# YoungSeng/QPGesture

Hardware: AMD Instinct MI355X
Metric: matched gesture frames/sec (GestureKNN) (higher is better)
Workload: dtype split-f16 products / f64 block sums + f64 re-evaluation; 1 GPU; 1 x 24 s clip (M=6 windows, Q=48 steps, 1440 frames each) per job vs speaker-10-class DB N_db=2048 windows (53248 candidates), shipped mode wavlm_feat(f32-bounded/f64-exact)+text(f32)+phase; n_db=2048, windows_per_clip=6, clips=1, clips_per_gpu=1, feature_dtype=f32, audio_precision=mixed, encode_batch=0, clips_in_flight=1, parallelism=single GPU, unsharded DB

## Files before the change

### include/qpg.h

```cpp
#ifndef QPG_H
#define QPG_H

#include <stddef.h>
#include <stdint.h>

#ifdef __cplusplus
extern "C" {
#endif

#define QPG_OK 0
#define QPG_EINVAL (-1)
#define QPG_EHIP (-2)
#define QPG_EUNSUP (-3)

typedef struct qpg_ctx qpg_ctx;

int qpg_version(void);
const char* qpg_build_id(void);
int qpg_ctx_create(int device, qpg_ctx** out);
int qpg_dev_kernarg(void);
int qpg_ctx_destroy(qpg_ctx* ctx);
#define QPG_OPT_GATE_DEDUP_FROM_CHAINS 0
#define QPG_OPT_TAKES_STAGES 1
#define QPG_OPT_NOPHASE_STAGES 2
// ... 8 lines not shown
int qpg_wavlm_resample_f32(qpg_ctx*, void* stream, const float* x, int64_t N, int Tin, int F, int Tout, float* out);

int qpg_frame_norm2_f64(qpg_ctx*, void* stream, const float* x, int64_t rows, int F, double* out);

int qpg_audio_cand_norm2(qpg_ctx*, void* stream, const double* fn2, int N, int T, const int32_t* cand_t,
                         int G, int n_taps, int tap_stride, double* cn2);

int qpg_l2_normalize_rows_f32(qpg_ctx*, void* stream, const float* x, int64_t rows, int D, float* out);
int qpg_text_pack_queries_f32(qpg_ctx*, void* stream, const float* x, int M, int R, int D, const int32_t* q_win,
                              const int32_t* q_row, int Q, float* out);


int qpg_audio_pack_queries(qpg_ctx*, void* stream, const float* qbase, int M, int T, int F,
                           const int32_t* q_win, const int32_t* q_t, int Q, int n_taps, int tap_stride,
                           float* q32, double* qn2);

int qpg_audio_cosine_f64(qpg_ctx*, void* stream, const float* base, int N, int T, int F,
                         const int32_t* cand_t, int G, int n_taps, int tap_stride, const double* cn2,
                         const float* q32, const double* qn2, int Q, double* D, int64_t ldD);
int qpg_audio_cosine_f64_h(qpg_ctx*, void* stream, const void* base_f16, int N, int T, int F,
                           const int32_t* cand_t, int G, int n_taps, int tap_stride, const double* cn2,
                           const float* q32, const double* qn2, int Q, double* D, int64_t ldD);

#define QPG_AUDIO_MX_ERR 2.05e-6
int qpg_audio_cosine_mx(qpg_ctx*, void* stream, const float* base, int N, int T, int F, const int32_t* cand_t, int G,
                        int n_taps, int tap_stride, const double* cn2, const float* q32, const double* qn2, int Q,
                        void* D, int d_is_f32, int64_t ldD, int32_t* stats);

int qpg_audio_cosine_mx_h(qpg_ctx*, void* stream, const void* base_f16, int N, int T, int F, const int32_t* cand_t, int G,
                          int n_taps, int tap_stride, const double* cn2, const float* q32, const double* qn2, int Q,
                          void* D, int d_is_f32, int64_t ldD, int32_t* stats);

#define QPG_AUDIO_HL_ERR 1.3e-6
int qpg_audio_hl_supported(int T, int F, int G, int n_taps, int tap_stride, int cand_step);
int qpg_audio_pack_queries_hl(qpg_ctx*, void* stream, const float* qbase, int M, int T, int F, const int32_t* q_win,
                              const int32_t* q_t, int Q, int n_taps, int tap_stride, float* q32, double* qn2, void* image,
                              int64_t image_bytes);
int64_t qpg_audio_hl_db_bytes(int N, int F);
int64_t qpg_audio_hl_query_bytes(int Q, int F);
int qpg_audio_hl_pack_db(qpg_ctx*, void* stream, const float* base, int N, int T, int F, int G, int n_taps, int tap_stride,
                         int cand_step, void* image, int64_t image_bytes);
int qpg_audio_hl_pack_queries(qpg_ctx*, void* stream, const float* q32, int Q, int F, void* image, int64_t image_bytes);
int qpg_clip_pack_hl(qpg_ctx*, void* stream, const float* qbase, int M, int T, int F, const int32_t* q_win,
                     const int32_t* q_t, int Q, int n_taps, int tap_stride, float* q32, double* qn2, void* image,
                     int64_t image_bytes, const float* text_ctx, int Mt, int R, int Dt, const int32_t* tq_win,
                     const int32_t* tq_row, int Qt, float* qn_out, void* cols_image, int64_t cols_bytes);
int qpg_audio_cosine_hl(qpg_ctx*, void* stream, const void* db_image, int N, int F, int G, const double* cn2,
                        const void* q_image, const double* qn2, int Q, void* D, int d_is_f32, int64_t ldD, int32_t* stats);
int qpg_audio_hl1_supported(int T, int F, int G, int n_taps, int tap_stride, int cand_step);
int64_t qpg_audio_hl1_db_bytes(int N, int F);
int qpg_audio_hl1_pack_db(qpg_ctx*, void* stream, const void* base_f16, int N, int T, int F, int G, int n_taps,
                          int tap_stride, int cand_step, void* image, int64_t image_bytes);
int qpg_audio_cosine_hl1(qpg_ctx*, void* stream, const void* db_image, int N, int F, int G, const double* cn2,
                         const void* q_image, const double* qn2, int Q, void* D, int d_is_f32, int64_t ldD, int32_t* stats);
int qpg_probe_mfma_f16_tile(qpg_ctx*, void* stream, const void* a, const void* b, const float* c, int tiles, float* out);

int qpg_text_pack_candidates_f32(qpg_ctx*, void* stream, const float* x, int N, int R, int Dm,
                                 const int32_t* cand_r, int G, float* xt);

int qpg_text_cosine_f32(qpg_ctx*, void* stream, const float* xt, int64_t C, int Dm, const float* qn, int Q,
                        float* D, int64_t ldD);

int64_t qpg_text_percode_ws_bytes(int64_t C, int Q, int K, int tiles_per_chunk);
int qpg_text_percode_f32(qpg_ctx*, void* stream, const float* xt, int64_t C, int Dm, const int16_t* cand_code, int K,
                         const float* qn, int Q, int tiles_per_chunk, int32_t idx_base, float absent, void* ws,
                         int64_t ws_bytes, float* out_dist, int32_t* out_idx, int16_t* out_rank, int32_t* out_nn);
int qpg_text_pack_candidates_f16(qpg_ctx*, void* stream, const float* x, int N, int R, int Dm, const int32_t* cand_r,
                                 int G, void* xh, float* nrm);
int qpg_text_percode_f16(qpg_ctx*, void* stream, const void* xh, const float* nrm, int64_t C, int Dm,
                         const int16_t* cand_code, int K, const float* qn, int Q, int32_t idx_base, float absent,
                         void* ws, int64_t ws_bytes, float* out_dist, int32_t* out_idx, int16_t* out_rank,
                         int32_t* out_nn);

int64_t qpg_hl_rows_bytes(int64_t R, int D);
int64_t qpg_hl_cols_bytes(int Q, int D);
int qpg_hl_pack_rows(qpg_ctx*, void* stream, const float* xs, int64_t R, int D, void* image, int64_t image_bytes);
int qpg_hl_pack_cols(qpg_ctx*, void* stream, const float* qn, int Q, int D, void* image, int64_t image_bytes);
int qpg_hl_prepare_queries(qpg_ctx*, void* stream, const float* q, int Q, int D, float* qn_out, void* cols_image,
                           int64_t image_bytes, float* qperm_out);
int qpg_hl_gemm_distance(qpg_ctx*, void* stream, const void* rows_image, int64_t R, int D, const void* cols_image, int Q,
                         float* Dm, int64_t ldD, float* tile_min, int64_t ldT);
int qpg_hl_gemm_tilemin(qpg_ctx*, void* stream, const void* rows_image, int64_t R, int D, const void* cols_image, int Q,
                        float band, float* tile_min, uint16_t* tile_mask, int64_t ldT);
int qpg_hl_gemm_tilemin_h(qpg_ctx*, void* stream, const void* rows_image, int64_t R, int D, const void* cols_image, int Q,
                          float band, float* tile_min_t, uint16_t* tile_mask_t, int64_t ldQ);
int qpg_perm32_rows_f32(qpg_ctx*, void* stream, const float* x, int64_t R, int D, float* y);
int qpg_percode_select_bycode_f32(qpg_ctx*, void* stream, const float* tile_min_t, const uint16_t* tile_mask_t, int64_t ldQ,
                                  int Q, int64_t R, const int16_t* row_code, const int32_t* row_index,
                                  const int32_t* zero_row, const int32_t* code_tile, int K, float band,
                                  const float* qn_perm, const float* xs_perm, int D, float absent, float* out_dist,
                                  int32_t* out_idx, int16_t* out_rank, int32_t* out_nn, int32_t* stats, int32_t idx_base);
int qpg_percode_select_sorted_f32(qpg_ctx*, void* stream, const float* Dm, int64_t ldD, const float* tile_min,
                                  const uint16_t* tile_mask , int64_t ldT,
                                  int Q, int64_t R, const int16_t* row_code, const int32_t* row_index,
                                  const int32_t* zero_row, const int32_t* code_tile, int K, float band, const float* qn,
                                  const float* xs, int D, float absent, float* out_dist, int32_t* out_idx,
                                  int16_t* out_rank, int32_t* out_nn, int32_t* stats, int32_t idx_base, int q_block,
                                  int64_t block_stride);

int qpg_wavvq_lev_f32(qpg_ctx*, void* stream, const int32_t* sym_db, int N, int T, const int32_t* cand_t, int G,
                      const int32_t* tap_off, int n_taps, const int32_t* sym_q, int Mq, int Tq,
                      const int32_t* q_win, const int32_t* q_t, int Q, float* D, int64_t ldD);

int qpg_percode_select_f64(qpg_ctx*, void* stream, const double* D, int64_t ldD, int Q, const int16_t* cand_code,
                           int64_t C, int K, double absent, int32_t idx_base, double* out_dist, int32_t* out_idx,
                           int16_t* out_rank, int q_block, int64_t block_stride);
int qpg_percode_select_f32(qpg_ctx*, void* stream, const float* D, int64_t ldD, int Q, const int16_t* cand_code,
                           int64_t C, int K, float absent, int32_t idx_base, float* out_dist, int32_t* out_idx,
                           int16_t* out_rank, int q_block, int64_t block_stride);

int qpg_percode_select_guarded_f64(qpg_ctx*, void* stream, const double* D, int64_t ldD, int Q, const int16_t* cand_code,
                                   int64_t C, int K, double absent, int32_t idx_base, double* out_dist, int32_t* out_idx,
                                   int16_t* out_rank, int q_block, int64_t block_stride, const float* base, int T, int F,
                                   const int32_t* cand_t, int G, int n_taps, int tap_stride, const float* q32, double eps,
                                   int32_t* stats, int base_is_f16);

int64_t qpg_percode_select_exact_ws_bytes(int Q, int64_t C, int K);
int qpg_percode_select_exact_f64(qpg_ctx*, void* stream, const double* D, int64_t ldD, int Q, const int16_t* cand_code,
                                 int64_t C, int K, double absent, int32_t idx_base, double* out_dist, int32_t* out_idx,
                                 int16_t* out_rank, int q_block, int64_t block_stride, const float* base, int T, int F,
                                 const int32_t* cand_t, int G, int n_taps, int tap_stride, const float* q32, double eps,
                                 int32_t* stats, int base_is_f16, void* ws, int64_t ws_bytes);

int qpg_percode_select_mixed_f64(qpg_ctx*, void* stream, const void* D, int d_is_f32, int64_t ldD, int Q, const int16_t* cand_code,
                                 int64_t C, int K, double absent, int32_t idx_base, double* out_dist, int32_t* out_idx,
                                 int16_t* out_rank, int q_block, int64_t block_stride, const float* base, int T, int F,
                                 const int32_t* cand_t, int G, int n_taps, int tap_stride, const float* q32,
                                 const double* qn2, const double* cn2, double eps1, double eps2, int32_t* stats,
                                 void* ws, int64_t ws_bytes, int base_is_f16);
int64_t qpg_percode_select_mixed_ws_bytes(int Q, int K);
int64_t qpg_percode_select_mixed_ws_stride(int K);
int qpg_percode_select_mixed_f64_cut(qpg_ctx*, void* stream, const void* D, int d_is_f32, int64_t ldD, int Q,
                                     const int16_t* cand_code, int64_t C, int K, double absent, int32_t idx_base,
                                     double* out_dist, int32_t* out_idx, int16_t* out_rank, int q_block, int64_t block_stride,
                                     const float* base, int T, int F, const int32_t* cand_t, int G, int n_taps,
                                     int tap_stride, const float* q32, const double* qn2, const double* cn2, double eps1,
                                     double eps2, int32_t* stats, void* ws, int64_t ws_bytes, int base_is_f16,
                                     const int16_t* pos_rank_t, const int16_t* freq_rank, int top_n, int probe);

int64_t qpg_merge_mixed_ws_bytes(int Q, int K, int fl_cap);
int qpg_merge_mixed_phase1_f64(qpg_ctx*, void* stream, const void* recv, int W, int64_t src_stride, int64_t dist_off,
                               int64_t idx_off, int Q, int K, double absent, double eps1, int R, void* req,
                               int64_t req_stride, void* ws, int64_t ws_bytes, int32_t* stats, int fl_cap,
                               int64_t flag_off);
int qpg_shard_refine_f64(qpg_ctx*, void* stream, const void* req_recv, int W, int64_t req_stride, int R, int q_stride,
                         int64_t cand_base, const float* base, int base_is_f16, int T, int F, const int32_t* cand_t, int G,
                         int n_taps, int tap_stride, const float* q32, const double* qn2, const double* cn2, void* resp,
                         int64_t resp_stride, int reference_arithmetic, int32_t* stats, int Rq);
int qpg_flags_stamp(qpg_ctx*, void* stream, void* buf, int nblk, int64_t stride, int64_t off, const int32_t* stats);
int qpg_flags_gather(qpg_ctx*, void* stream, const void* buf, int nblk, int64_t stride, int64_t off, int32_t* stats);
int qpg_merge_mixed_phase2_f64(qpg_ctx*, void* stream, const void* recv, int W, int64_t src_stride, int64_t idx_off, int Q,
                               int K, double absent, const void* ws, int64_t ws_bytes, const void* resp_recv,
                               int64_t resp_stride, double* out_dist, int32_t* out_idx, int16_t* out_rank, int32_t* stats,
                               int fl_cap, double eps2);

int qpg_merge_select_f64(qpg_ctx*, void* stream, const void* recv, int W, int64_t src_stride, int64_t dist_off,
                         int64_t idx_off, int Q, int K, double absent, double* out_dist, int32_t* out_idx,
                         int16_t* out_rank, double eps2, int32_t* stats);
int qpg_merge_select_f32(qpg_ctx*, void* stream, const void* recv, int W, int64_t src_stride, int64_t dist_off,
                         int64_t idx_off, int Q, int K, float absent, float* out_dist, int32_t* out_idx,
                         int16_t* out_rank);

int qpg_rank_rows_f64(qpg_ctx*, void* stream, const double* d, int Q, int K, int16_t* out);
int qpg_rank_rows_f32(qpg_ctx*, void* stream, const float* d, int Q, int K, int16_t* out);


// ... 365 lines not shown
```

### qpgesture_amd/csrc/qpg_audio_hl.hip

```cpp
#include "qpg_common.h"
#include <stdlib.h>

typedef _Float16 h8 __attribute__((ext_vector_type(8)));
typedef _Float16 h4 __attribute__((ext_vector_type(4)));

#define HL_ROWS 27
#define HL_SUB 3
#define HL_QC 48
#define HL_CT 6
#define HL_GQC (16 * HL_CT)
#define HL_KS 2
#define HL_PIECE 1024

template <int PJ>
__device__ __forceinline__ float xor_lanes_f(float v) {
  return __int_as_float(lane_xor<PJ>(__float_as_int(v)));
}
__device__ __forceinline__ f32x4 mfma_h(h8 a, h8 b, f32x4 c) {
  return __builtin_amdgcn_mfma_f32_16x16x32_f16(a, b, c, 0, 0, 0);
}

__device__ __forceinline__ void split_hl(float x, _Float16& h, _Float16& l) {
  h = (_Float16)x;
  const float r = x - (float)h;
// ... 220 lines not shown

__global__ __launch_bounds__(768) void hl_pack_queries_fused_kernel(const float* __restrict__ qbase, int M, int T, int F,
                                                                    const int32_t* __restrict__ q_win,
                                                                    const int32_t* __restrict__ q_t, int Q, int tap_stride,
                                                                    float* __restrict__ q32, double* __restrict__ qn2,
                                                                    _Float16* __restrict__ image,
                                                                    int32_t* __restrict__ qexp) {
  hl_pack_query_block(blockIdx.x, threadIdx.x, qbase, M, T, F, q_win, q_t, Q, tap_stride, q32, qn2, image, qexp);
}

struct ClipPackText {
  const float* ctx;
  const int32_t* q_win;
  const int32_t* q_row;
  int R, Dt, Qt;
  float* qn;
  _Float16* image;
  int32_t* qexp;
};

__global__ __launch_bounds__(768) void hl_pack_clip_kernel(const float* __restrict__ qbase, int M, int T, int F,
                                                           const int32_t* __restrict__ q_win,
                                                           const int32_t* __restrict__ q_t, int Q, int tap_stride,
                                                           float* __restrict__ q32, double* __restrict__ qn2,
                                                           _Float16* __restrict__ image, int32_t* __restrict__ qexp,
                                                           int n_aud, ClipPackText tx) {
  const int tid = threadIdx.x;
  if ((int)blockIdx.x < n_aud) {
    hl_pack_query_block(blockIdx.x, tid, qbase, M, T, F, q_win, q_t, Q, tap_stride, q32, qn2, image, qexp);
    return;
  }
  const int qi = (int)blockIdx.x - n_aud;
  const int D = tx.Dt;
  extern __shared__ __attribute__((aligned(16))) float rowbuf[];
  __shared__ float n_s;
  const bool live = qi < tx.Qt;
  const float* p = live ? tx.ctx + ((int64_t)tx.q_win[qi] * tx.R + tx.q_row[qi]) * D : tx.ctx;
  if (tid < 4) {
    const float n = einsum_norm_f32(p, D, tid);
    if (tid == 0) n_s = n;
  }
  __syncthreads();
  const float n = n_s;
  float m = 0.f;
  for (int e = tid; e < D; e += 768) {
    const float v = live ? f_div(p[e], n) : 0.f;
    rowbuf[e] = v;
    if (live) tx.qn[(int64_t)qi * D + e] = v;
    m = fmaxf(m, fabsf(v));
  }
  const int e_q = hl_block_exponent<12>(m);
  if (live && tid == 0) tx.qexp[qi] = e_q;
  const float sc = ldexpf(1.0f, e_q);
  const int KB = D / 32, K8 = D / 8;
  for (int k8 = tid; k8 < K8; k8 += 768) {
    const int k = k8 * 8;
    h8 hh, ll;
    hl_split8<false>(rowbuf + k, sc, hh, ll);
    hl_store_col_piece(tx.image, qi, HL_GQC, KB, k, 0, hh, ll);
  }
}

struct HlArgs {
  const _Float16* db;
  const _Float16* qi;
  const int32_t* meta;
  const int32_t* qexp;
  const double* cn2;
  const double* qn2;
  void* D;
  const float* zeros;
  int64_t ldD;
  int32_t* stats;
  int N, G, Q, KB, d_f32;
  int j0;
  int chunks;
  float* tmin;
  int64_t ldT;
  uint16_t* tmask;
  float band;
};

#define HL_RING (2 * HL_KS)
#define HL_PS (3 * HL_KS)

#define HL_PD 1
#define HL_WPB 4
#define HL_MINW 2
#define HL_THREADS (128 * HL_WPB)
#define HL_SGB(mask, n) __builtin_amdgcn_sched_group_barrier(mask, n, 0)
__global__ __launch_bounds__(HL_THREADS, HL_MINW) void hl_gemm16_kernel(HlArgs a) {
  extern __shared__ __attribute__((aligned(16))) unsigned char lds[];
  const int tid = threadIdx.x, lane = tid & 63, w = tid >> 6;
  const int wl = w >> 1, t = w & 1;
  const int xl = (int)blockIdx.x, slot = xl >> 3;
  const int wgrp = (slot / a.chunks) * 8 + (xl & 7);
  const int chunk = slot % a.chunks;
  if (a.j0 + wgrp * HL_WPB >= a.N) return;
  const int j = a.j0 + wgrp * HL_WPB + wl;
  const int KB = a.KB, n_stage = KB / HL_KS;
  const bool win_ok = j < a.N;
  const bool row_ok = win_ok;
  const int64_t unit0 = (((int64_t)j * 2 + t) * KB * 2) * 64 + lane;
  const h8* dbp = row_ok ? reinterpret_cast<const h8*>(a.db) + unit0 : reinterpret_cast<const h8*>(a.zeros);
  const int pl_step = row_ok ? 64 : 0;
  const int kb_step = 2 * pl_step;
  auto load_a = [&](int kb, h8 (&dst)[2]) {
    dst[0] = dbp[(int64_t)kb * kb_step];
    dst[1] = dbp[(int64_t)kb * kb_step + pl_step];
  };
  constexpr int stage_units = HL_KS * HL_CT * 2 * 64;
  const h8* qsrc = reinterpret_cast<const h8*>(a.qi) + (int64_t)chunk * KB * HL_CT * 2 * 64;
  constexpr int QLD = stage_units / HL_THREADS;
  h8 qreg[QLD];
  auto load_q = [&](int s) {
    s = s < n_stage ? s : n_stage - 1;
#pragma unroll
    for (int u = 0; u < QLD; ++u) qreg[u] = qsrc[(int64_t)s * stage_units + u * HL_THREADS + tid];
  };
  auto store_q = [&](int buf) {
    h8* dst = reinterpret_cast<h8*>(lds) + buf * stage_units;
#pragma unroll
    for (int u = 0; u < QLD; ++u) dst[u * HL_THREADS + tid] = qreg[u];
  };
  auto lds_barrier = [&]() {
    asm volatile("s_waitcnt lgkmcnt(0)" ::: "memory");
    __builtin_amdgcn_s_barrier();
  };

  double acc[HL_CT][4];
  f32x4 xacc[HL_CT];
#pragma unroll
  for (int c = 0; c < HL_CT; ++c) {
    xacc[c] = (f32x4){0.f, 0.f, 0.f, 0.f};
#pragma unroll
    for (int r = 0; r < 4; ++r) acc[c][r] = 0.0;
  }
  h8 ring[HL_RING][2];
#pragma unroll
  for (int i = 0; i < HL_RING; ++i) load_a(i, ring[i]);
  load_q(0);
  store_q(0);
  load_q(1);
  lds_barrier();
  store_q(1);
  load_q(2);
  const f32x4 zero4 = (f32x4){0.f, 0.f, 0.f, 0.f};
  h8 B[HL_PD + 1][2][2];
  auto ld_b = [&](int buf, int ps, h8 (&d)[2][2]) {
    const h8* qb = reinterpret_cast<const h8*>(lds) + buf * stage_units + lane;
    const int k2 = ps / 3, c0 = 2 * (ps % 3);
#pragma unroll
    for (int jj = 0; jj < 2; ++jj)
#pragma unroll
      for (int pl = 0; pl < 2; ++pl) d[jj][pl] = qb[((k2 * HL_CT + c0 + jj) * 2 + pl) * 64];
  };
  f32x4 hp[2] = {zero4, zero4};
  f32x4 hold[HL_CT];
  static_assert(HL_KS == 2, "the h h' chains pair the two k-blocks of a stage");
#pragma unroll
  for (int i = 0; i < HL_PD; ++i) ld_b(0, i, B[i]);

  for (int s2 = 0; s2 < n_stage; s2 += 2) {
#pragma unroll
    for (int ss = 0; ss < 2; ++ss) {
      const int s = s2 + ss;
#pragma unroll
      for (int ps = 0; ps < HL_PS; ++ps) {
        const int k2 = ps / 3, c0 = 2 * (ps % 3);
        const int pc0 = 2 * ((ps + 2) % 3);
        const int kb = s * HL_KS + k2;
        h8 (&af)[2] = ring[(ss * HL_KS + k2) % HL_RING];
        h8 (&Bc)[2][2] = B[(ss * HL_PS + ps) % (HL_PD + 1)];
        h8 (&Bn)[2][2] = B[(ss * HL_PS + ps + HL_PD) % (HL_PD + 1)];
        if (ps == HL_PS - HL_PD) {
          lds_barrier();
        }
        if (ps >= HL_PS - HL_PD) ld_b((ss + 1) & 1, ps + HL_PD - HL_PS, Bn);
        else ld_b(ss, ps + HL_PD, Bn);
        const f32x4 h0 = mfma_h(af[0], Bc[0][0], k2 == 0 ? zero4 : hold[c0]);
        const f32x4 h1 = mfma_h(af[0], Bc[1][0], k2 == 0 ? zero4 : hold[c0 + 1]);
        xacc[c0] = mfma_h(af[0], Bc[0][1], xacc[c0]);
        xacc[c0 + 1] = mfma_h(af[0], Bc[1][1], xacc[c0 + 1]);
        xacc[c0] = mfma_h(af[1], Bc[0][0], xacc[c0]);
        xacc[c0 + 1] = mfma_h(af[1], Bc[1][0], xacc[c0 + 1]);
        if (((ps + HL_PS - 1) % HL_PS) / 3 == HL_KS - 1) {
#pragma unroll
          for (int jj = 0; jj < 2; ++jj)
#pragma unroll
            for (int r = 0; r < 4; ++r) acc[pc0 + jj][r] += (double)hp[jj][r];
        }
        if (k2 == 0) {
          hold[c0] = h0;
          hold[c0 + 1] = h1;
        } else {
          hp[0] = h0;
          hp[1] = h1;
        }
        if (ps % 3 == 2) {
          const int kn = kb + HL_RING < KB ? kb + HL_RING : KB - 1;
          load_a(kn, af);
        }
        if (ps == HL_PS - 1) {
          store_q(ss);
          load_q(s + 3);
        }
#pragma unroll
        for (int i = 0; i < 6; ++i) {
          HL_SGB(0x008, 1);
          if (i < 4) HL_SGB(0x100, 1);
          HL_SGB(0x002, 3);
        }
      }
    }
  }
#pragma unroll
  for (int jj = 0; jj < 2; ++jj)
#pragma unroll
    for (int r = 0; r < 4; ++r) acc[4 + jj][r] += (double)hp[jj][r];
  asm volatile("s_waitcnt vmcnt(0) lgkmcnt(0)" ::: "memory");
  __builtin_amdgcn_s_barrier();

  const int cg = lane & 15, rg = lane >> 4;
  if (!win_ok) return;
  const int e_c1 = a.meta[0];
#pragma unroll
  for (int ct = 0; ct < HL_CT; ++ct) {
    const int q = chunk * (16 * HL_CT) + ct * 16 + cg;
    if (q >= a.Q) continue;
    const int e_q1 = a.qexp[q];
    f32x4 o;
#pragma unroll
    for (int r = 0; r < 4; ++r)
      o[r] = (float)(1.0 - ldexp(acc[ct][r] + (double)xacc[ct][r] * (1.0 / 2048.0), -(e_c1 + e_q1)));
    if (a.D)
      *reinterpret_cast<f32x4*>(reinterpret_cast<float*>(a.D) + (int64_t)q * a.ldD + (int64_t)j * 32 + 16 * t + 4 * rg) = o;
    if (a.tmin) {
      float m = fminf(fminf(o[0], o[1]), fminf(o[2], o[3]));
      m = fminf(m, xor_lanes_f<16>(m));
      m = fminf(m, xor_lanes_f<32>(m));
      if (rg == 0) a.tmin[(int64_t)q * a.ldT + (int64_t)j * 2 + t] = m;
      if (a.tmask) {
        const float lim = m + a.band;
        unsigned int bits = ((o[0] <= lim) ? 1u : 0u) | ((o[1] <= lim) ? 2u : 0u) | ((o[2] <= lim) ? 4u : 0u) |
                            ((o[3] <= lim) ? 8u : 0u);
        bits <<= 4 * rg;
        bits |= (unsigned int)lane_xor<16>((int)bits);
        bits |= (unsigned int)lane_xor<32>((int)bits);
        if (rg == 0) a.tmask[(int64_t)q * a.ldT + (int64_t)j * 2 + t] = (uint16_t)bits;
      }
    }
  }
}


__device__ __forceinline__ double fast_rsqrt_f64(double x) {
  const float xf = (float)x;
  double y = (double)__builtin_amdgcn_rsqf(xf);
  const double hx = 0.5 * x;
  y = y * (1.5 - hx * y * y);
  y = y * (1.5 - hx * y * y);
  return y;
}
#define H2_W 8
#define H2_RS2 2
template <int PL, int RS, bool NT>
__global__ __launch_bounds__(64 * H2_W, 2) void audio_cosine_hl2_kernel(HlArgs a) {
  extern __shared__ __attribute__((aligned(16))) unsigned char lds[];
  const int tid = threadIdx.x, lane = tid & 63, w = tid >> 6;
  const int xl = (int)blockIdx.x, slot = xl >> 3;
  const int wgrp = (slot / a.chunks) * 8 + (xl & 7);
  const int chunk = slot % a.chunks;
  if (a.j0 + wgrp * H2_W >= a.N) return;
  const int j = a.j0 + wgrp * H2_W + w;
  const bool win_ok = j < a.N;
  const int KB = a.KB, n_stage = KB / 2;
  const int cg = lane & 15, rg = lane >> 4;
  const int jb = a.j0 + wgrp * H2_W;
  const uint32_t wj = (uint32_t)(win_ok ? w : a.N - 1 - jb);
  const uint32_t win_units = (uint32_t)(PL == 2 ? HL_WIN_UNITS(KB) : HL1_WIN_UNITS(KB));
  const unsigned char* sbase = reinterpret_cast<const unsigned char*>(a.db) + (int64_t)jb * win_units * 16;
  const uint32_t o0 = (wj * win_units + (uint32_t)lane) * 16u;
  const uint32_t o1 = (wj * win_units + (uint32_t)KB * (64 * PL) + 11u * rg + (cg < 11 ? cg : 10)) * 16u;
  constexpr uint32_t st0 = 64u * PL * 16u, st1 = (uint32_t)PL * HL_T1_UNITS * 16u;
  auto ld_frag = [](const unsigned char* p) -> h8 {
    if (NT) return __builtin_nontemporal_load(reinterpret_cast<const h8*>(p));
    return *reinterpret_cast<const h8*>(p);
  };
  auto load_a = [&](int kb, h8 (&d)[2 * PL]) {
    kb = kb < KB ? kb : KB - 1;
    const uint32_t a0 = o0 + (uint32_t)kb * st0, a1 = o1 + (uint32_t)kb * st1;
    d[0] = ld_frag(sbase + a0);
    if (PL == 2) d[1] = ld_frag(sbase + a0 + 64 * 16);
    d[PL] = ld_frag(sbase + a1);
    if (PL == 2) d[PL + 1] = ld_frag(sbase + a1 + HL_T1_UNITS * 16);
  };
  constexpr int stage_units = 2 * HL_CT * 2 * 64;
  constexpr int QLD = stage_units / (64 * H2_W);
  const unsigned char* qsrc = reinterpret_cast<const unsigned char*>(a.qi) + (int64_t)chunk * KB * HL_CT * 2 * 1024;
  const uint32_t qoff = (uint32_t)tid * 16u;
  h8 qreg[QLD];
  auto load_q = [&](int s) {
    s = s < n_stage ? s : n_stage - 1;
#pragma unroll
    for (int u = 0; u < QLD; ++u)
      qreg[u] = *reinterpret_cast<const h8*>(qsrc + (int64_t)s * (stage_units * 16) + u * (64 * H2_W * 16) + qoff);
  };
  auto store_q = [&](int buf) {
    h8* dst = reinterpret_cast<h8*>(lds) + buf * stage_units;
#pragma unroll
// ... 844 lines not shown
          if (c == CT - 1) load_a(rf_base, rf_t, (uint32_t)k2 * rf_k, Ac);
          if (st == 0) HL_SGB(0x020, QLD);
          if (st == NS - G64_PD) HL_SGB(0x200, QLD);
          HL_SGB(0x008, 1);
          HL_SGB(0x100, 1);
          HL_SGB(0x008, 3);
          if (c == CT - 1) HL_SGB(0x020, 4);
        }
      }
    }
    const Rows done = cur;
    const int chunk = it_cur.ch;
    cur = nxt;
    it_cur = it_nxt;
    if (done.ok) epilogue(done, chunk);
    if (!more) break;
  }
  asm volatile("s_waitcnt vmcnt(0) lgkmcnt(0)" ::: "memory");
}

QPG_HOOK_VAR(int, g_gemm64_nw, 4);
#ifdef QPG_DEBUG_HOOKS
extern "C" int qpg_debug_gemm64_waves(int nw) {
  QPG_REQUIRE(nw == 4 || nw == 8, "qpg_debug_gemm64_waves: 4 or 8");
  g_gemm64_nw = nw;
  return QPG_OK;
}
#endif

static HlArgs hl_gemm_args(qpg_ctx* ctx, const void* rows_image, int64_t R, int D, const void* cols_image, int Q, float* Dm,
                           int64_t ldD, float* tile_min, int64_t ldT, uint16_t* tile_mask, float band) {
  const HlColsView cv = hl_cols_view(cols_image, Q, D);
  HlArgs a;
  a.db = static_cast<const _Float16*>(rows_image);
  a.meta = hl_rows_meta(rows_image, R, D);
  a.qi = cv.frags;
  a.qexp = cv.qexp;
  a.cn2 = nullptr; a.qn2 = nullptr; a.D = Dm; a.zeros = ctx->zeros; a.ldD = ldD; a.stats = nullptr;
  a.N = (int)(R / 32); a.j0 = 0; a.chunks = cv.chunks; a.G = 0; a.Q = Q; a.KB = D / 32; a.d_f32 = 1;
  a.tmin = tile_min; a.ldT = ldT; a.tmask = tile_mask; a.band = band;
  return a;
}

extern "C" int qpg_hl_gemm_tilemin_h(qpg_ctx* ctx, void* stream, const void* rows_image, int64_t R, int D,
                                     const void* cols_image, int Q, float band, float* tile_min, uint16_t* tile_mask,
                                     int64_t ldQ) {
  const char* name = "qpg_hl_gemm_tilemin_h";
  QPG_REQUIRE(ctx && rows_image && cols_image && tile_min && tile_mask, "%s: null pointer", name);
  QPG_REQUIRE(R > 0 && (R % 64) == 0 && R / 32 < 0x7fffffff && Q > 0 && D > 0 && (D % 128) == 0 && ldQ >= Q && band >= 0.f,
              "%s: bad size (R %% 64 == 0, D %% 128 == 0, ldQ >= Q, band >= 0)", name);
  const HlArgs a = hl_gemm_args(ctx, rows_image, R, D, cols_image, Q, nullptr, 0, tile_min, ldQ, tile_mask, band);
  const int chunks = a.chunks, KB = a.KB;
  const size_t lds64 = 2 * (size_t)G64_KS * HL_CT * HL_PIECE;
  static bool raised64 = false;
  if (!raised64) {
    bool ok = true;
#define G64_RAISE(P_, W_) ok = ok && hipFuncSetAttribute(reinterpret_cast<const void*>(hl_gemm64h_kernel<HL_CT, P_, W_>), \
                                                         hipFuncAttributeMaxDynamicSharedMemorySize, (int)lds64) == hipSuccess
    G64_RAISE(true, 8); G64_RAISE(false, 8); G64_RAISE(true, 4); G64_RAISE(false, 4);
#undef G64_RAISE
    if (!ok) {
      qpg_set_error("%s: cannot raise the dynamic LDS limit", name);
      return QPG_EHIP;
    }
    raised64 = true;
  }
  const int nw = g_gemm64_nw;
  const int64_t g8 = (R / 64 + nw - 1) / nw;
  QPG_REQUIRE(g8 * chunks < 0x7fffffffll, "%s: too many work items", name);
  const int n_items = (int)(g8 * chunks);
  const int slots = ctx->n_cu * (8 / nw);
  const int n_blocks = n_items < slots ? n_items : slots;
  const bool pair = (KB / G64_KS) % 2 == 0;
#define G64_GO(P_, W_) hipLaunchKernelGGL((hl_gemm64h_kernel<HL_CT, P_, W_>), dim3(n_blocks), dim3(64 * W_), lds64, qpg_stream(stream), a, n_items)
  if (nw == 8) { if (pair) G64_GO(true, 8); else G64_GO(false, 8); }
  else { if (pair) G64_GO(true, 4); else G64_GO(false, 4); }
#undef G64_GO
  QPG_LAUNCH_CHECK("hl_gemm64h_kernel");
  return QPG_OK;
}

static int hl_gemm_impl(const char* name, qpg_ctx* ctx, void* stream, const void* rows_image, int64_t R, int D,
                        const void* cols_image, int Q, float* Dm, int64_t ldD, float* tile_min, int64_t ldT,
                        uint16_t* tile_mask, float band) {
  QPG_REQUIRE(ctx && rows_image && cols_image && (Dm || (tile_min && tile_mask)), "%s: null pointer", name);
  QPG_REQUIRE(R > 0 && (R % 32) == 0 && R / 32 < 0x7fffffff && Q > 0 && D > 0 && (D % 128) == 0 &&
                  (!Dm || (ldD >= R && (ldD % 4) == 0 && (reinterpret_cast<uintptr_t>(Dm) % 16) == 0)),
              "%s: bad size (R %% 32 == 0, D %% 128 == 0, ldD %% 4 == 0, 16-byte aligned output)", name);
  QPG_REQUIRE(!tile_min || ldT >= R / 16, "%s: tile_min needs ldT >= R / 16", name);
  QPG_REQUIRE(!tile_mask || (tile_min && band >= 0.f), "%s: tile masks need the tile minima and a band >= 0", name);
  const HlArgs a = hl_gemm_args(ctx, rows_image, R, D, cols_image, Q, Dm, ldD, tile_min, ldT, tile_mask, band);
  const int chunks = a.chunks, KB = a.KB;
  if ((KB % G32_RING) == 0 && Q > 48) {
    const size_t lds32 = 2 * (size_t)G32_KS * HL_CT * 2 * HL_PIECE;
    static bool raised32 = false;
    if (!raised32) {
      if (hipFuncSetAttribute(reinterpret_cast<const void*>(hl_gemm32_kernel<6>), hipFuncAttributeMaxDynamicSharedMemorySize,
                              (int)lds32) != hipSuccess) {
        qpg_set_error("%s: cannot raise the dynamic LDS limit", name);
        return QPG_EHIP;
      }
      raised32 = true;
    }
    const int64_t g8 = (a.N + 7) / 8;
    QPG_REQUIRE(g8 * chunks < 0x7fffffffll, "%s: too many work items", name);
    const int n_items = (int)(g8 * chunks);
    const int n_blocks = n_items < ctx->n_cu ? n_items : ctx->n_cu;
    hipLaunchKernelGGL(hl_gemm32_kernel<6>, dim3(n_blocks), dim3(512), lds32, qpg_stream(stream), a, n_items);
    QPG_LAUNCH_CHECK("hl_gemm32_kernel");
    return QPG_OK;
  }
  const size_t lds_bytes = 2 * HL_KS * HL_CT * 2 * HL_PIECE;
  const int64_t rgroups = (a.N + HL_WPB - 1) / HL_WPB;
  QPG_REQUIRE(((rgroups + 7) / 8) * 8 * chunks < 0x7fffffffll, "%s: too many blocks", name);
  hipLaunchKernelGGL(hl_gemm16_kernel, dim3((unsigned)(((rgroups + 7) / 8) * 8 * chunks)), dim3(HL_THREADS),
                     lds_bytes, qpg_stream(stream), a);
  QPG_LAUNCH_CHECK("hl_gemm16_kernel");
  return QPG_OK;
}

extern "C" int qpg_hl_gemm_distance(qpg_ctx* ctx, void* stream, const void* rows_image, int64_t R, int D,
                                    const void* cols_image, int Q, float* Dm, int64_t ldD, float* tile_min, int64_t ldT) {
  return hl_gemm_impl("qpg_hl_gemm_distance", ctx, stream, rows_image, R, D, cols_image, Q, Dm, ldD, tile_min, ldT, nullptr,
                      0.f);
}

extern "C" int qpg_hl_gemm_tilemin(qpg_ctx* ctx, void* stream, const void* rows_image, int64_t R, int D,
                                   const void* cols_image, int Q, float band, float* tile_min, uint16_t* tile_mask,
                                   int64_t ldT) {
  return hl_gemm_impl("qpg_hl_gemm_tilemin", ctx, stream, rows_image, R, D, cols_image, Q, nullptr, 0, tile_min, ldT,
                      tile_mask, band);
}

__global__ __launch_bounds__(64) void hl_probe_kernel(const _Float16* __restrict__ A, const _Float16* __restrict__ B,
                                                      const float* __restrict__ C, float* __restrict__ out) {
  const int tile = blockIdx.x, lane = threadIdx.x;
  const h8 a = reinterpret_cast<const h8*>(A + (int64_t)tile * 512 + (lane & 15) * 32)[lane >> 4];
  const h8 b = reinterpret_cast<const h8*>(B + (int64_t)tile * 512 + (lane & 15) * 32)[lane >> 4];
  f32x4 c = (f32x4){0.f, 0.f, 0.f, 0.f};
  if (C)
#pragma unroll
    for (int r = 0; r < 4; ++r) c[r] = C[(int64_t)tile * 256 + (4 * (lane >> 4) + r) * 16 + (lane & 15)];
  const f32x4 d = mfma_h(a, b, c);
#pragma unroll
  for (int r = 0; r < 4; ++r) out[(int64_t)tile * 256 + (4 * (lane >> 4) + r) * 16 + (lane & 15)] = d[r];
}

extern "C" int qpg_probe_mfma_f16_tile(qpg_ctx* ctx, void* stream, const void* a, const void* b, const float* c, int tiles,
                                       float* out) {
  QPG_REQUIRE(ctx && a && b && out && tiles > 0, "qpg_probe_mfma_f16_tile: bad argument");
  hipLaunchKernelGGL(hl_probe_kernel, dim3(tiles), dim3(64), 0, qpg_stream(stream), static_cast<const _Float16*>(a),
                     static_cast<const _Float16*>(b), c, out);
  QPG_LAUNCH_CHECK("hl_probe_kernel");
  return QPG_OK;
}
```

Before: 5.612 million frames/s.

## Template hl_gemm16 kernel on live column tiles to skip empty query tiles

Makes the 16-row split-f16 GEMM kernel a template over the number of 16-query column tiles. When there is a single chunk with Q ≤ 48, it launches with only the tiles that hold queries. The pair-step schedule, LDS staging and accumulator folding are generalised so that a pair can span two k-blocks or share one tile. This is meant to cut the MFMA work, LDS and registers spent on padded query columns. It also adds a public qpg_hl_gemm16 entry point that forces this path over the 32-row kernel. The trade-off is more complex indexing, and the wider kernel may or may not be on the default call path.

Result: slower. 5.533 million frames/s (-1.4%).

```diff
diff --git a/include/qpg.h b/include/qpg.h
--- a/include/qpg.h
+++ b/include/qpg.h
@@ -114,6 +114,8 @@
                          float* Dm, int64_t ldD, float* tile_min, int64_t ldT);
 int qpg_hl_gemm_tilemin(qpg_ctx*, void* stream, const void* rows_image, int64_t R, int D, const void* cols_image, int Q,
                         float band, float* tile_min, uint16_t* tile_mask, int64_t ldT);
+int qpg_hl_gemm16(qpg_ctx*, void* stream, const void* rows_image, int64_t R, int D, const void* cols_image, int Q,
+                  float* Dm, int64_t ldD, float band, float* tile_min, uint16_t* tile_mask, int64_t ldT);
 int qpg_hl_gemm_tilemin_h(qpg_ctx*, void* stream, const void* rows_image, int64_t R, int D, const void* cols_image, int Q,
                           float band, float* tile_min_t, uint16_t* tile_mask_t, int64_t ldQ);
 int qpg_perm32_rows_f32(qpg_ctx*, void* stream, const float* x, int64_t R, int D, float* y);
diff --git a/qpgesture_amd/csrc/qpg_audio_hl.hip b/qpgesture_amd/csrc/qpg_audio_hl.hip
--- a/qpgesture_amd/csrc/qpg_audio_hl.hip
+++ b/qpgesture_amd/csrc/qpg_audio_hl.hip
@@ -326,15 +326,16 @@
 };
 
 #define HL_RING (2 * HL_KS)
-#define HL_PS (3 * HL_KS)
 
 #define HL_PD 1
 #define HL_WPB 4
 #define HL_MINW 2
 #define HL_THREADS (128 * HL_WPB)
 #define HL_SGB(mask, n) __builtin_amdgcn_sched_group_barrier(mask, n, 0)
+template <int CT>
 __global__ __launch_bounds__(HL_THREADS, HL_MINW) void hl_gemm16_kernel(HlArgs a) {
   extern __shared__ __attribute__((aligned(16))) unsigned char lds[];
+  constexpr int PS = HL_KS * CT / 2;
   const int tid = threadIdx.x, lane = tid & 63, w = tid >> 6;
   const int wl = w >> 1, t = w & 1;
   const int xl = (int)blockIdx.x, slot = xl >> 3;
@@ -353,29 +354,46 @@
     dst[0] = dbp[(int64_t)kb * kb_step];
     dst[1] = dbp[(int64_t)kb * kb_step + pl_step];
   };
-  constexpr int stage_units = HL_KS * HL_CT * 2 * 64;
+  constexpr int stage_units = HL_KS * CT * 2 * 64;
+  constexpr int kb_units = CT * 2 * 64;
   const h8* qsrc = reinterpret_cast<const h8*>(a.qi) + (int64_t)chunk * KB * HL_CT * 2 * 64;
-  constexpr int QLD = stage_units / HL_THREADS;
+  constexpr int QLD = (stage_units + HL_THREADS - 1) / HL_THREADS;
+  static_assert(QLD * HL_THREADS <= 2 * stage_units, "a surplus unit wraps round once");
   h8 qreg[QLD];
+  auto q_unit = [&](int u) {
+    const int v = u * HL_THREADS + tid;
+    return v >= stage_units ? v - stage_units : v;
+  };
   auto load_q = [&](int s) {
     s = s < n_stage ? s : n_stage - 1;
 #pragma unroll
-    for (int u = 0; u < QLD; ++u) qreg[u] = qsrc[(int64_t)s * stage_units + u * HL_THREADS + tid];
+    for (int u = 0; u < QLD; ++u) {
+      if constexpr (CT == HL_CT) {
+        qreg[u] = qsrc[(int64_t)s * stage_units + u * HL_THREADS + tid];
+      } else {
+        static_assert(HL_KS == 2, "a stage's units are two runs of the image");
+        const int v = q_unit(u), k2 = v >= kb_units ? 1 : 0;
+        qreg[u] = qsrc[((int64_t)s * HL_KS + k2) * (HL_CT * 2 * 64) + (v - k2 * kb_units)];
+      }
+    }
   };
   auto store_q = [&](int buf) {
     h8* dst = reinterpret_cast<h8*>(lds) + buf * stage_units;
 #pragma unroll
-    for (int u = 0; u < QLD; ++u) dst[u * HL_THREADS + tid] = qreg[u];
+    for (int u = 0; u < QLD; ++u) {
+      if constexpr (CT == HL_CT) dst[u * HL_THREADS + tid] = qreg[u];
+      else dst[q_unit(u)] = qreg[u];
+    }
   };
   auto lds_barrier = [&]() {
     asm volatile("s_waitcnt lgkmcnt(0)" ::: "memory");
     __builtin_amdgcn_s_barrier();
   };
 
-  double acc[HL_CT][4];
-  f32x4 xacc[HL_CT];
-#pragma unroll
-  for (int c = 0; c < HL_CT; ++c) {
+  double acc[CT][4];
+  f32x4 xacc[CT];
+#pragma unroll
+  for (int c = 0; c < CT; ++c) {
     xacc[c] = (f32x4){0.f, 0.f, 0.f, 0.f};
 #pragma unroll
     for (int r = 0; r < 4; ++r) acc[c][r] = 0.0;
@@ -393,15 +411,15 @@
   h8 B[HL_PD + 1][2][2];
   auto ld_b = [&](int buf, int ps, h8 (&d)[2][2]) {
     const h8* qb = reinterpret_cast<const h8*>(lds) + buf * stage_units + lane;
-    const int k2 = ps / 3, c0 = 2 * (ps % 3);
 #pragma unroll
     for (int jj = 0; jj < 2; ++jj)
 #pragma unroll
-      for (int pl = 0; pl < 2; ++pl) d[jj][pl] = qb[((k2 * HL_CT + c0 + jj) * 2 + pl) * 64];
+      for (int pl = 0; pl < 2; ++pl) d[jj][pl] = qb[((2 * ps + jj) * 2 + pl) * 64];
   };
   f32x4 hp[2] = {zero4, zero4};
-  f32x4 hold[HL_CT];
+  f32x4 hold[CT];
   static_assert(HL_KS == 2, "the h h' chains pair the two k-blocks of a stage");
+  static_assert((2 * PS) % (HL_PD + 1) == 0, "a trip's pair-steps must keep the fragment ring's index static");
 #pragma unroll
   for (int i = 0; i < HL_PD; ++i) ld_b(0, i, B[i]);
 
@@ -410,42 +428,57 @@
     for (int ss = 0; ss < 2; ++ss) {
       const int s = s2 + ss;
 #pragma unroll
-      for (int ps = 0; ps < HL_PS; ++ps) {
-        const int k2 = ps / 3, c0 = 2 * (ps % 3);
-        const int pc0 = 2 * ((ps + 2) % 3);
-        const int kb = s * HL_KS + k2;
-        h8 (&af)[2] = ring[(ss * HL_KS + k2) % HL_RING];
-        h8 (&Bc)[2][2] = B[(ss * HL_PS + ps) % (HL_PD + 1)];
-        h8 (&Bn)[2][2] = B[(ss * HL_PS + ps + HL_PD) % (HL_PD + 1)];
-        if (ps == HL_PS - HL_PD) {
+      for (int ps = 0; ps < PS; ++ps) {
+        const int k0 = (2 * ps) / CT, c0 = (2 * ps) % CT;
+        const int k1 = (2 * ps + 1) / CT, c1 = (2 * ps + 1) % CT;
+        const int pp = (ps + PS - 1) % PS;
+        h8 (&af0)[2] = ring[(ss * HL_KS + k0) % HL_RING];
+        h8 (&af1)[2] = ring[(ss * HL_KS + k1) % HL_RING];
+        h8 (&Bc)[2][2] = B[(ss * PS + ps) % (HL_PD + 1)];
+        h8 (&Bn)[2][2] = B[(ss * PS + ps + HL_PD) % (HL_PD + 1)];
+        if (ps == PS - HL_PD) {
           lds_barrier();
         }
-        if (ps >= HL_PS - HL_PD) ld_b((ss + 1) & 1, ps + HL_PD - HL_PS, Bn);
+        if (ps >= PS - HL_PD) ld_b((ss + 1) & 1, ps + HL_PD - PS, Bn);
         else ld_b(ss, ps + HL_PD, Bn);
-        const f32x4 h0 = mfma_h(af[0], Bc[0][0], k2 == 0 ? zero4 : hold[c0]);
-        const f32x4 h1 = mfma_h(af[0], Bc[1][0], k2 == 0 ? zero4 : hold[c0 + 1]);
-        xacc[c0] = mfma_h(af[0], Bc[0][1], xacc[c0]);
-        xacc[c0 + 1] = mfma_h(af[0], Bc[1][1], xacc[c0 + 1]);
-        xacc[c0] = mfma_h(af[1], Bc[0][0], xacc[c0]);
-        xacc[c0 + 1] = mfma_h(af[1], Bc[1][0], xacc[c0 + 1]);
-        if (((ps + HL_PS - 1) % HL_PS) / 3 == HL_KS - 1) {
+        f32x4 h0, h1;
+        if (c0 != c1) {
+          h0 = mfma_h(af0[0], Bc[0][0], k0 == 0 ? zero4 : hold[c0]);
+          h1 = mfma_h(af1[0], Bc[1][0], k1 == 0 ? zero4 : hold[c1]);
+          xacc[c0] = mfma_h(af0[0], Bc[0][1], xacc[c0]);
+          xacc[c1] = mfma_h(af1[0], Bc[1][1], xacc[c1]);
+          xacc[c0] = mfma_h(af0[1], Bc[0][0], xacc[c0]);
+          xacc[c1] = mfma_h(af1[1], Bc[1][0], xacc[c1]);
+        } else {
+          h0 = mfma_h(af0[0], Bc[0][0], zero4);
+          h1 = mfma_h(af1[0], Bc[1][0], h0);
+          xacc[c0] = mfma_h(af0[0], Bc[0][1], xacc[c0]);
+          xacc[c0] = mfma_h(af0[1], Bc[0][0], xacc[c0]);
+          xacc[c0] = mfma_h(af1[0], Bc[1][1], xacc[c0]);
+          xacc[c0] = mfma_h(af1[1], Bc[1][0], xacc[c0]);
+        }
+        if ((2 * pp) / CT == HL_KS - 1) {
 #pragma unroll
           for (int jj = 0; jj < 2; ++jj)
 #pragma unroll
-            for (int r = 0; r < 4; ++r) acc[pc0 + jj][r] += (double)hp[jj][r];
-        }
-        if (k2 == 0) {
-          hold[c0] = h0;
-          hold[c0 + 1] = h1;
-        } else {
-          hp[0] = h0;
-          hp[1] = h1;
-        }
-        if (ps % 3 == 2) {
-          const int kn = kb + HL_RING < KB ? kb + HL_RING : KB - 1;
-          load_a(kn, af);
-        }
-        if (ps == HL_PS - 1) {
+            for (int r = 0; r < 4; ++r) acc[(2 * pp + jj) % CT][r] += (double)hp[jj][r];
+        } else if ((2 * pp + 1) / CT == HL_KS - 1) {
+#pragma unroll
+          for (int r = 0; r < 4; ++r) acc[(2 * pp + 1) % CT][r] += (double)hp[1][r];
+        }
+        if (k0 == 0) hold[c0] = h0;
+        else hp[0] = h0;
+        if (k1 == 0) hold[c1] = h1;
+        else hp[1] = h1;
+        if (c0 == CT - 1) {
+          const int kb = s * HL_KS + k0, kn = kb + HL_RING < KB ? kb + HL_RING : KB - 1;
+          load_a(kn, af0);
+        }
+        if (c1 == CT - 1) {
+          const int kb = s * HL_KS + k1, kn = kb + HL_RING < KB ? kb + HL_RING : KB - 1;
+          load_a(kn, af1);
+        }
+        if (ps == PS - 1) {
           store_q(ss);
           load_q(s + 3);
         }
@@ -458,10 +491,15 @@
       }
     }
   }
-#pragma unroll
-  for (int jj = 0; jj < 2; ++jj)
-#pragma unroll
-    for (int r = 0; r < 4; ++r) acc[4 + jj][r] += (double)hp[jj][r];
+  if constexpr (CT > 1) {
+#pragma unroll
+    for (int jj = 0; jj < 2; ++jj)
+#pragma unroll
+      for (int r = 0; r < 4; ++r) acc[CT - 2 + jj][r] += (double)hp[jj][r];
+  } else {
+#pragma unroll
+    for (int r = 0; r < 4; ++r) acc[0][r] += (double)hp[1][r];
+  }
   asm volatile("s_waitcnt vmcnt(0) lgkmcnt(0)" ::: "memory");
   __builtin_amdgcn_s_barrier();
 
@@ -469,7 +507,7 @@
   if (!win_ok) return;
   const int e_c1 = a.meta[0];
 #pragma unroll
-  for (int ct = 0; ct < HL_CT; ++ct) {
+  for (int ct = 0; ct < CT; ++ct) {
     const int q = chunk * (16 * HL_CT) + ct * 16 + cg;
     if (q >= a.Q) continue;
     const int e_q1 = a.qexp[q];
@@ -1480,7 +1518,7 @@
 
 static int hl_gemm_impl(const char* name, qpg_ctx* ctx, void* stream, const void* rows_image, int64_t R, int D,
                         const void* cols_image, int Q, float* Dm, int64_t ldD, float* tile_min, int64_t ldT,
-                        uint16_t* tile_mask, float band) {
+                        uint16_t* tile_mask, float band, bool rows16 = false) {
   QPG_REQUIRE(ctx && rows_image && cols_image && (Dm || (tile_min && tile_mask)), "%s: null pointer", name);
   QPG_REQUIRE(R > 0 && (R % 32) == 0 && R / 32 < 0x7fffffff && Q > 0 && D > 0 && (D % 128) == 0 &&
                   (!Dm || (ldD >= R && (ldD % 4) == 0 && (reinterpret_cast<uintptr_t>(Dm) % 16) == 0)),
@@ -1489,7 +1527,7 @@
   QPG_REQUIRE(!tile_mask || (tile_min && band >= 0.f), "%s: tile masks need the tile minima and a band >= 0", name);
   const HlArgs a = hl_gemm_args(ctx, rows_image, R, D, cols_image, Q, Dm, ldD, tile_min, ldT, tile_mask, band);
   const int chunks = a.chunks, KB = a.KB;
-  if ((KB % G32_RING) == 0 && Q > 48) {
+  if ((KB % G32_RING) == 0 && Q > 48 && !rows16) {
     const size_t lds32 = 2 * (size_t)G32_KS * HL_CT * 2 * HL_PIECE;
     static bool raised32 = false;
     if (!raised32) {
@@ -1508,11 +1546,18 @@
     QPG_LAUNCH_CHECK("hl_gemm32_kernel");
     return QPG_OK;
   }
-  const size_t lds_bytes = 2 * HL_KS * HL_CT * 2 * HL_PIECE;
   const int64_t rgroups = (a.N + HL_WPB - 1) / HL_WPB;
   QPG_REQUIRE(((rgroups + 7) / 8) * 8 * chunks < 0x7fffffffll, "%s: too many blocks", name);
-  hipLaunchKernelGGL(hl_gemm16_kernel, dim3((unsigned)(((rgroups + 7) / 8) * 8 * chunks)), dim3(HL_THREADS),
-                     lds_bytes, qpg_stream(stream), a);
+  const int live = chunks == 1 && Q <= 48 ? (Q + 15) / 16 : HL_CT;
+#define HL16_GO(CT_) hipLaunchKernelGGL(hl_gemm16_kernel<CT_>, dim3((unsigned)(((rgroups + 7) / 8) * 8 * chunks)),       \
+                                        dim3(HL_THREADS), 2 * (size_t)HL_KS * CT_ * 2 * HL_PIECE, qpg_stream(stream), a)
+  switch (live) {
+    case 1: HL16_GO(1); break;
+    case 2: HL16_GO(2); break;
+    case 3: HL16_GO(3); break;
+    default: HL16_GO(HL_CT); break;
+  }
+#undef HL16_GO
   QPG_LAUNCH_CHECK("hl_gemm16_kernel");
   return QPG_OK;
 }
@@ -1528,6 +1573,12 @@
                                    int64_t ldT) {
   return hl_gemm_impl("qpg_hl_gemm_tilemin", ctx, stream, rows_image, R, D, cols_image, Q, nullptr, 0, tile_min, ldT,
                       tile_mask, band);
+}
+
+extern "C" int qpg_hl_gemm16(qpg_ctx* ctx, void* stream, const void* rows_image, int64_t R, int D, const void* cols_image,
+                             int Q, float* Dm, int64_t ldD, float band, float* tile_min, uint16_t* tile_mask, int64_t ldT) {
+  return hl_gemm_impl("qpg_hl_gemm16", ctx, stream, rows_image, R, D, cols_image, Q, Dm, ldD, tile_min, ldT, tile_mask,
+                      tile_mask ? band : 0.f, true);
 }
 
 __global__ __launch_bounds__(64) void hl_probe_kernel(const _Float16* __restrict__ A, const _Float16* __restrict__ B,
```
